# shanpenghui/ExtractORB

Measured on AMD Instinct MI355X. Metric: frames/sec (ORB extract, 640x480x8-level x1000 feat), higher is better.
Workload: dtype u8; 1 GPU; mono640: 640x480 mono stream, 8 levels, 1000 features, synthetic noise frames; variant=noise, nfeatures=1000, nlevels=8, handles_per_gpu=1, parallelism=frames sharded 512/GPU

## Files before the change

### extractorb_amd/csrc/k_pyramid.hip

```cpp
#include <hip/hip_runtime.h>
#include <stdint.h>

#include "orbx_device.hpp"

namespace orbx {

__device__ __forceinline__ int reflect101(int p, int n) {
    p = p < 0 ? -p : p;
    return p >= n ? 2 * (n - 1) - p : p;
}

constexpr int kPyrRows = kResizeTileRows / 4;
constexpr int kTileCols = 64;
constexpr int kTileRowGroups = 4;
constexpr int kTileRows = kPyrRows * kTileRowGroups;

static __host__ __device__ inline int rowDwords(const LevelGeom& g) { return (kPadL - kEdge + g.w + 2 * kEdge + 3) / 4; }

struct SrcView {
    const uint8_t* p;
    long long frame;
    int stride;
    int readableCols;
    int aligned;
};

__device__ __forceinline__ unsigned mulHi24(unsigned a, unsigned b) {
    unsigned r;
    asm("v_mul_hi_u32_u24 %0, %1, %2" : "=v"(r) : "v"(a), "v"(b));
    return r;
}
__device__ __forceinline__ unsigned pkLshr2(unsigned a) {
    unsigned r;
    asm("v_pk_lshrrev_b16 %0, %2, %1" : "=v"(r) : "v"(a), "s"(0x00020002u));
    return r;
}
typedef unsigned short u16x2 __attribute__((ext_vector_type(2)));

template <bool PACKED>
__device__ __forceinline__ void resizeTile(const SrcView& sv, const LevelGeom& d, const ResizeX* __restrict__ xt, const QuadRec* __restrict__ xq,
                                           const ResizeX* __restrict__ yt, const TileFoot ft, uint8_t* __restrict__ pyr,
                                           int tileX, int tileY, int f, uint8_t* tile, int ldsStride) {
    const int tid = threadIdx.x, col = tid & (kTileCols - 1), rgrp = tid / kTileCols;
    const int nd = rowDwords(d), wB = d.w + 2 * kEdge;
// ... 171 lines not shown
extern "C" int orbx_debug_chain_stamps(unsigned long long* out32) { return (int)hipMemcpyFromSymbol(out32, HIP_SYMBOL(g_chainStamps), sizeof(unsigned long long) * 32); }
__device__ unsigned long long g_chainSpans[3 * 2048];
extern "C" int orbx_debug_chain_spans(unsigned long long* out) { return (int)hipMemcpyFromSymbol(out, HIP_SYMBOL(g_chainSpans), sizeof(g_chainSpans)); }
#define CSPAN_BEGIN do { if (tid == 0 && t < 2048) g_chainSpans[3 * t] = __builtin_amdgcn_s_memrealtime(); } while (0)
#define CSPAN_END(lvl) do { if (tid == 0 && t < 2048) { g_chainSpans[3 * t + 1] = __builtin_amdgcn_s_memrealtime(); g_chainSpans[3 * t + 2] = (unsigned long long)(lvl); } } while (0)
#else
#define CSTAMP(i) do {} while (0)
#define CSPAN_BEGIN do {} while (0)
#define CSPAN_END(lvl) do {} while (0)
#endif

template <int T>
__device__ __forceinline__ void chainStep(const uint8_t* S, uint8_t* D, const ChainRegion rs, const ChainRegion rd, const ChainDeal dl, const ResizeX* qrs, const ResizeX* cys,
                                          const int ss, const int ds, const int tid) {
    static_assert(T == 256 || T == 512, "PyrColumn::deal holds the dealing for 256 and 512 deriving threads");
    const int nq = (rd.w + 3) >> 2, nb = dl.nb, blk = (int)(((unsigned)tid * dl.recip) >> 20), x4 = 4 * (tid - blk * nq);
    const int per = dl.per, yb = blk * per, ye = min(yb + per, (int)rd.h);
    if (blk < nb && yb < ye) {
        u16x2 wt[4];
        unsigned sel[4];
        const uint4* qr = (const uint4*)((const QuadRec*)qrs + (x4 >> 2));
        const uint4 q0 = qr[0], q1 = qr[1];
        const unsigned bs = ((const unsigned*)qr)[8];
        sel[0] = q0.x; sel[1] = q0.y; sel[2] = q0.z; sel[3] = q0.w;
        wt[0] = __builtin_bit_cast(u16x2, q1.x); wt[1] = __builtin_bit_cast(u16x2, q1.y); wt[2] = __builtin_bit_cast(u16x2, q1.z); wt[3] = __builtin_bit_cast(u16x2, q1.w);
        const int base = (int)(bs & 0xffffu);
        const unsigned sh = bs >> 16;
        auto hrow = [&](int srow, unsigned (&h)[4]) {
            const unsigned* rp = (const unsigned*)(S + __mul24(srow - rs.y0, ss) + base);
            const unsigned p0 = rp[0], p1 = rp[1], p2 = rp[2];
            const unsigned P0 = __builtin_amdgcn_alignbyte(p1, p0, sh), P1 = __builtin_amdgcn_alignbyte(p2, p1, sh);
#pragma unroll
            for (int k = 0; k < 4; k++)
                h[k] = __builtin_amdgcn_udot2(__builtin_bit_cast(u16x2, __builtin_amdgcn_perm(P1, P0, sel[k])), wt[k], 0u, false) & ~15u;
        };
        unsigned HA[4] = {0, 0, 0, 0}, HB[4] = {0, 0, 0, 0};
// ... 1 lines not shown
        const RowRec* rrs = (const RowRec*)cys;
        for (int y = yb; y < ye; y++) {
            const RowRec rr = rrs[y];
            if (rr.sA != haveA) { hrow(rr.sA, HA); haveA = rr.sA; }
            if (rr.sB != haveB) { hrow(rr.sB, HB); haveB = rr.sB; }
            unsigned t[4];
#pragma unroll
            for (int k = 0; k < 4; k++) t[k] = mulHi24(rr.bA, HA[k]) + mulHi24(rr.bB, HB[k]) + 2u;
            const unsigned u01 = pkLshr2(t[0] | (t[1] << 16)), u23 = pkLshr2(t[2] | (t[3] << 16));
            *(unsigned*)(D + y * ds + x4) = __builtin_amdgcn_perm(u23, u01, 0x06040200u);
        }
    }
}

template <bool PACKED, int T, int TD>
__global__ __launch_bounds__(T) void k_pyr_cols(SrcView img, const PyrColumn* __restrict__ cols, const ColLevels* __restrict__ lvp, int nlevels,
                                                            const ResizeX* __restrict__ colCoef, int coefSlot,
                                                            uint8_t* __restrict__ pyr, int bufEvenBytes, int f0, int nFrames) {
    static_assert(TD <= T && TD % 64 == 0 && (T - TD) % 64 == 0, "roles are whole waves");
    extern __shared__ __align__(16) uint8_t lds[];
    __shared__ __align__(16) ResizeX coef[kChainCoefMax];
    struct LevelOut { ColOwn own; int w, h, stride; long long off; };
    __shared__ LevelOut outOf[kMaxLevels];
    int t, fr;
    if (!xcdChunkFrame(nFrames, t, fr)) return;
    const int f = f0 + fr, tid = threadIdx.x;
    const PyrColumn& pc = cols[t];
    const ColLevels& lv = *lvp;
    const int top = nlevels - 1;
    LevelOut myOut{};
    if (tid < nlevels) myOut = LevelOut{pc.own[tid], lv.w[tid], lv.h[tid], lv.pyrStride[tid], lv.pyrOff[tid] + (long long)f * lv.pyrFrameBytes[tid]};
    CSTAMP(0);
    CSPAN_BEGIN;
    auto bufOf = [&](int j) { return lds + ((j & 1) ? bufEvenBytes : 0); };
    constexpr int kStatic = 8;
    ChainRegion rj[kStatic + 1];
#pragma unroll
    for (int j = 0; j <= kStatic; j++) rj[j] = pc.region[j];
    {
        const ChainRegion r = rj[0];
        const int nDw = r.w >> 2, total = nDw * r.h;
        const uint8_t* src = img.p + (long long)f * img.frame + (long long)r.y0 * img.stride + r.x0;
        unsigned* dst = (unsigned*)bufOf(0);
        constexpr int kLoads = (kChainMaxH0 * kChainMaxW / 4 + T - 1) / T;
        const float inv = __frcp_rn((float)nDw);
        unsigned w[kLoads];
#pragma unroll
        for (int i = 0; i < kLoads; i++) {
            w[i] = 0;
            if (i * T < total) {
            const int idx = min(tid + i * T, total - 1);
            const int row = (int)(((float)idx + 0.5f) * inv), c = idx - row * nDw;
            const uint8_t* q = src + ((unsigned)__mul24(row, img.stride) + 4u * (unsigned)c);
            const int x = r.x0 + 4 * c;
            if (img.aligned && x >= 0 && x + 3 < img.readableCols) w[i] = *(const unsigned*)q;
            else {
#pragma unroll
                for (int b = 0; b < 4; b++) w[i] |= (unsigned)q[reflect101(x + b, img.readableCols) - x] << (8 * b);
            }
            }
        }
        constexpr int kPerThread = (kChainCoefMax + T - 1) / T;
        const int nCoef = pc.nCoef;
        const ResizeX* mine = colCoef + (size_t)t * (size_t)coefSlot;
        ResizeX cv[kPerThread];
#pragma unroll
        for (int k = 0; k < kPerThread; k++) cv[k] = tid + k * T < nCoef ? mine[tid + k * T] : ResizeX{0, 0, 0, 0};
#pragma unroll
        for (int k = 0; k < kPerThread; k++)
            if (tid + k * T < nCoef) coef[tid + k * T] = cv[k];
        if (tid < nlevels) outOf[tid] = myOut;
#pragma unroll
        for (int i = 0; i < kLoads; i++)
            if (tid + i * T < total) dst[tid + i * T] = w[i];
    }
    __syncthreads();
    CSTAMP(1);
    int off = 0;
    auto doLevel = [&](const int j, const ChainRegion rs, const ChainRegion rd) {
        const int ss = (rs.w + 3) & ~3;
        const uint8_t* S = bufOf(j);
        constexpr int TW = TD < T ? T - TD : T;
        if (j < top) {
            const ResizeX* cxs = coef + off;
            const int nqUnits = 6 * ((rd.w + 3) >> 2);
            if (tid < TD) chainStep<TD>(S, bufOf(j + 1), rs, rd, pc.deal[TD == 512][j + 1 < kMaxLevels ? j + 1 : j], cxs, cxs + nqUnits, ss, (rd.w + 3) & ~3, tid);
            off += nqUnits + 2 * rd.h;
        }
        const bool everyone = TD == T || j == top;
        const int wtid = everyone ? tid : tid - TD, wstep = everyone ? T : TW;
        if (wtid >= 0) {
        const LevelOut lo = outOf[j];
        const ColOwn own = lo.own;
        const int w = lo.w, h = lo.h, wB = w + 2 * kEdge;
        uint8_t* out = pyr + lo.off;
        const int stride = lo.stride, nrows = own.r1 - own.r0;
        const int fa = max((int)own.dw0, kPadL / 4), fb = max(fa, min((int)own.dw1, kPadL / 4 + (w >> 2)));
        if (fb > fa && (fb - fa) * nrows <= 2 * wstep) {
            const int ndw = fb - fa, total = ndw * nrows;
            const float inv = __frcp_rn((float)ndw);
            for (int i = wtid; i < total; i += wstep) {
                const int rr = (int)(((float)i + 0.5f) * inv), dw = fa + (i - rr * ndw), row = own.r0 + rr;
                const uint8_t* srow = S + __mul24(reflect101(row - kEdge, h) - rs.y0, ss) - rs.x0;
                *(unsigned*)(out + (long long)row * stride + 4 * dw) = *(const unsigned*)(srow + (4 * dw - kPadL));
            }
        } else if (fb > fa) {
            const int ndw = fb - fa;
            const float rdw = __frcp_rn((float)ndw);
            const int ngrp = max((int)(((float)wstep + 0.5f) * rdw), 1);
            const int per = (int)(((float)(nrows + ngrp - 1) + 0.5f) * __frcp_rn((float)ngrp));
            const int grp = (int)(((float)wtid + 0.5f) * rdw), c = wtid - grp * ndw;
            if (wtid >= 0 && grp < ngrp) {
                const int rA = own.r0 + grp * per, rB = min(rA + per, (int)own.r1);
                const uint8_t* scol = S + (4 * (fa + c) - kPadL - rs.x0);
                uint8_t* ocol = out + 4 * (fa + c);
                auto run = [&](const int r0, const int r1, const int src0, const int sstep) {
                    const uint8_t* sp = scol + __mul24(src0 - rs.y0, ss);
                    uint8_t* op = ocol + (long long)r0 * stride;
                    for (int row = r0; row < r1; row++, op += stride, sp += sstep) *(unsigned*)op = *(const unsigned*)sp;
                };
                const int t1 = min(rB, kEdge), m0 = max(rA, kEdge), m1 = min(rB, kEdge + h), b0 = max(rA, kEdge + h);
                if (rA < t1) run(rA, t1, kEdge - rA, -ss);
                if (m0 < m1) run(m0, m1, m0 - kEdge, ss);
                if (b0 < rB) run(b0, rB, 2 * (h - 1) - (b0 - kEdge), -ss);
            }
        }
        const int nL = fa - own.dw0, nO = nL + (own.dw1 - fb);
        if (nO > 0) {
            const int total = nO * nrows;
            const float inv = __frcp_rn((float)nO);
            for (int i = wtid; i < total; i += wstep) {
                const int rr = (int)(((float)i + 0.5f) * inv), jj = i - rr * nO, dw = jj < nL ? own.dw0 + jj : fb + (jj - nL), row = own.r0 + rr;
                const uint8_t* srow = S + __mul24(reflect101(row - kEdge, h) - rs.y0, ss) - rs.x0;
                const int bc0 = 4 * dw;
                unsigned o = 0;
#pragma unroll
                for (int k = 0; k < 4; k++) {
                    int bx = bc0 + k - (kPadL - kEdge);
                    bx = bx < 0 ? 0 : (bx > wB - 1 ? wB - 1 : bx);
                    o |= (unsigned)srow[reflect101(bx - kEdge, w)] << (8 * k);
                }
                *(unsigned*)(out + (long long)row * stride + bc0) = o;
            }
        }
        }
        __syncthreads();
        CSTAMP(j + 2);
    };
#pragma unroll
    for (int j = 0; j < kStatic; j++)
        if (j <= top) doLevel(j, rj[j], rj[j + 1]);
    for (int j = kStatic; j <= top; j++) doLevel(j, pc.region[j], pc.region[j + 1 < kMaxLevels ? j + 1 : j]);
    CSPAN_END(0);
}

void launchPyrCols(hipStream_t st, const uint8_t* img, long long stride, long long frameStride, int imgW, const PyrColumn* cols, int nCols,
                   const ColLevels* lv, int nlevels, const ResizeX* colCoef, int coefSlot, uint8_t* pyr, int ldsBytes, int bufEvenBytes,
                   bool packed, int shape, int f0, int B) {
    SrcView sv;
    sv.p = img; sv.stride = (int)stride; sv.frame = frameStride; sv.readableCols = imgW;
    sv.aligned = (((uintptr_t)img | (uintptr_t)stride | (uintptr_t)frameStride) & 3) == 0;
#define ORBX_COLS_LAUNCH(P, T, TD) hipLaunchKernelGGL((k_pyr_cols<P, T, TD>), xcdGrid(nCols, B), dim3(T), (size_t)ldsBytes, st, sv, cols, lv, nlevels, colCoef, coefSlot, \
                                                  pyr, bufEvenBytes, f0, B)
    (void)packed;
    if (shape == 6) ORBX_COLS_LAUNCH(true, 1024, 512);
    else if (shape == 4) ORBX_COLS_LAUNCH(true, 768, 256);
    else ORBX_COLS_LAUNCH(true, 512, 256);
#undef ORBX_COLS_LAUNCH
}

void launchPyrFirst(hipStream_t st, const uint8_t* img, long long stride, long long frameStride, const LevelGeom& g0,
                    const LevelGeom* g1, int tilesX0, int tilesY0, int tilesX1, int tilesY1, const ResizeX* xt, const QuadRec* xq,
                    const ResizeX* yt, const TileFoot* foot, uint8_t* pyr, int ldsStride, int ldsRows, bool packed, int f0, int B) {
    SrcView sv;
    sv.p = img; sv.stride = (int)stride; sv.frame = frameStride; sv.readableCols = g0.w;
    sv.aligned = (((uintptr_t)img | (uintptr_t)stride | (uintptr_t)frameStride) & 3) == 0;
    const int n0 = tilesX0 * tilesY0, n1 = g1 ? tilesX1 * tilesY1 : 0;
// ... 15 lines not shown
```

### extractorb_amd/csrc/orbx_api.cpp

```cpp
#include "orbx_internal.hpp"

static_assert(sizeof(orbx_keypoint) == sizeof(Keypoint), "orbx_keypoint layout");
static_assert(sizeof(orbx_proj_query) == sizeof(ProjQuery), "orbx_proj_query layout");

double g_hostT[8];
long g_hostN;
const bool g_hostTiming = getenv("ORBX_HOST_TIMING") && atoi(getenv("ORBX_HOST_TIMING")) != 0;
TestAids g_aids;
const char* const kSlotNames[ORBX_NUM_KERNELS] = {"k_pyr_first", "k_resize", "k_blur", "k_fast",
                                            "k_octree", "k_describe", "memset+copies", "batch_total",
                                            "k_stereo_rows+match+filter", "k_frame_finish+k_search_init+k_search_proj"};
thread_local std::string g_createError;

namespace {
void freeAll(orbx_handle* h) {
    void* dev[] = {h->d_input, h->d_pyr, h->d_blur, h->d_candPos, h->d_candSeg, h->d_cellCount, h->d_cellOff, h->d_nodeOf, h->d_candCount, h->d_sink, h->d_sel, h->d_levelCount,
                   h->d_levelLap, h->d_lap, h->d_lv, h->d_cells, h->d_rx, h->d_ry, h->d_xq, h->d_cols, h->d_colLevels, h->d_colCoef, h->d_foot, h->d_tiles, h->d_laneItem, h->d_out,
                   h->d_octArena, h->d_leafHist, h->d_leafBest, h->d_leafCode, h->d_bowWord, h->d_bowNode, h->d_bowWeight, h->d_rowOff, h->d_sadDist,
                   h->d_nMatched, h->d_rowList, h->d_uRight, h->d_depth, h->d_clock, h->d_sim3Rec, h->d_frustumCounts, h->twoViewWork.prep, h->twoViewWork.first,
                   h->twoViewWork.second, h->twoViewWork.score, h->twoViewWork.mats, h->twoViewWork.inl, h->twoViewWork.counted, h->twoViewWork.cosv, h->sim3SolveWork.prep,
                   h->sim3SolveWork.idx1, h->sim3SolveWork.pts, h->sim3SolveWork.counts, h->sim3SolveWork.its};
    for (void* p : dev) if (p) (void)hipFree(p);
    if (h->evFork) (void)hipEventDestroy(h->evFork);
    if (h->evJoin) (void)hipEventDestroy(h->evJoin);
    if (h->aux) (void)hipStreamDestroy(h->aux);
    if (h->aux2) (void)hipStreamDestroy(h->aux2);
    if (h->probeStream) { (void)hipStreamSynchronize(h->probeStream); (void)hipStreamDestroy(h->probeStream); }
    for (int i = 0; i < 2; i++) { if (h->evPyr[i]) (void)hipEventDestroy(h->evPyr[i]); if (h->evBlur[i]) (void)hipEventDestroy(h->evBlur[i]); if (h->evUp[i]) (void)hipEventDestroy(h->evUp[i]); }
    void* host[] = {h->h_lap, h->h_out, h->h_in, h->h_pyr, h->h_tab};
    for (void* p : host) if (p) (void)hipHostFree(p);
    for (auto& ev : h->pending) { (void)hipEventDestroy(ev.a); (void)hipEventDestroy(ev.b); }
    if (h->ownStream && h->stream) (void)hipStreamDestroy(h->stream);
// ... 55 lines not shown
    stage(h->d_lv, g.lv, sizeof(LevelGeom) * g.nlevels);
    stage(h->d_cells, g.cells.data(), sizeof(CellDesc) * g.cells.size());
    size_t fo = 0;
    for (int l = 1; l < g.nlevels; l++) {
        footOff[l] = fo;
        if (fo + g.foot[l].size() > h->footCap) return fail(h, ORBX_ERR_IMAGE_TOO_LARGE, "tile footprint table does not fit");
        stage(h->d_foot + fo, g.foot[l].data(), sizeof(TileFoot) * g.foot[l].size());
        fo += g.foot[l].size();
    }
    {
        size_t n = 0, nc = 0;
        for (FrameGeom::ColumnSet& cs : g.colSets) {
            if (n + cs.columns.size() > h->colsCap || nc + cs.coef.size() > h->colCoefCap) cs.fit = false;
            if (!cs.fit) continue;
            stage(h->d_cols + n, cs.columns.data(), sizeof(PyrColumn) * cs.columns.size());
            stage(h->d_colCoef + nc, cs.coef.data(), sizeof(ResizeX) * cs.coef.size());
            const size_t slot = &cs - g.colSets.data();
            colsOff[slot] = n;
            colCoefOff[slot] = nc;
            n += cs.columns.size();
            nc += cs.coef.size();
        }
        ColLevels c{};
        c.nlevels = g.nlevels;
        for (int l = 0; l < g.nlevels; l++) {
            c.w[l] = g.lv[l].w; c.h[l] = g.lv[l].h; c.pyrStride[l] = g.lv[l].pyrStride; c.rxOff[l] = g.lv[l].rxOff; c.ryOff[l] = g.lv[l].ryOff;
            c.pyrOff[l] = g.lv[l].pyrOff; c.pyrFrameBytes[l] = g.lv[l].pyrFrameBytes;
        }
        stage(h->d_colLevels, &c, sizeof(c));
    }
// ... 76 lines not shown
    auto pollute = [&](hipStream_t st) { if (h->ldsPollute >= 0) launchLdsPollute(st, lp.numCUs, h->ldsPollute, h->d_sink); };
    auto blurTable = [&](hipStream_t st, int v, int blockRows, int f0, int Bn) {
        launchBlur(st, h->d_tiles + gp.blurItemOff[v], h->d_laneItem + gp.blurLaneOff[v], gp.nBlurLanes[v], blockRows, h->d_lv, h->d_pyr, h->d_blur, f0, Bn);
    };
    bool blurJoin[2] = {false, false};
    int blurF0[2] = {0, 0}, blurBn[2] = {0, 0};
    auto front = [&](hipStream_t st, int f0, int Bn) {
        const FrontPlan fp = planFront(g, gp, lp, state, bp, Bn);
        h->lastPyrCut = fp.cut >= 0 ? g.colSets[fp.cut].px : 0;
        h->lastPyrForm = fp.pyrForm();
        if (fp.cut >= 0) {
            const FrameGeom::ColumnSet& cs = g.colSets[fp.cut];
            Prof p(h, S_RESIZE, st);
            h->lastKernel[S_RESIZE] = fp.resizeKernel;
            pollute(st);
            launchPyrCols(st, d_imgs, stride, frameStride, g.lv[0].w, h->d_cols + h->colsOff[fp.cut], (int)cs.columns.size(), h->d_colLevels, g.nlevels,
                          h->d_colCoef + h->colCoefOff[fp.cut], cs.coefSlot, h->d_pyr, cs.ldsBytes, cs.evenBytes,
                          g.colsPacked && !lp.resizeBytewise, fp.colsShape, f0, Bn);
        } else {
            {
                Prof p(h, S_LEVEL0, st);
                pollute(st);
                launchPyrFirst(st, d_imgs, stride, frameStride, g.lv[0], g.nlevels > 1 ? &g.lv[1] : nullptr, g.tilesX[0], g.tilesY[0],
                               g.tilesX[1], g.tilesY[1], h->d_rx + h->rxOff[1], h->d_xq + h->xqOff[1], h->d_ry + h->ryOff[1], h->d_foot + h->footOff[1], h->d_pyr,
                               g.tileLdsStride, g.tileLdsRows, g.packedTaps[1] && !lp.resizeBytewise, f0, Bn);
            }
            for (int l = 2; l < g.nlevels; l++) {
                Prof p(h, S_RESIZE, st);
                h->lastKernel[S_RESIZE] = fp.resizeKernel;
                pollute(st);
                launchResize(st, g.lv[l - 1], g.lv[l], g.tilesX[l], g.tilesY[l], h->d_rx + h->rxOff[l], h->d_xq + h->xqOff[l], h->d_ry + h->ryOff[l],
// ... 332 lines not shown
    h->colPx = envInt("ORBX_PYR_COL_PX", 0);
    h->launch.fastWide = envInt("ORBX_FAST_WIDE", -1);
    h->launch.patchBlur = envInt("ORBX_PATCH_BLUR", -1);
    h->launch.blurSplit = envInt("ORBX_BLUR_SPLIT", -1);
    h->sharedUploadBytes = g_aids.sharedUploadBytes;
    h->twoEyesWalk = g_aids.twoEyesWalk == 1;
    h->describeSums = g_aids.describeSums == 0 || g_aids.describeSums == 1 ? g_aids.describeSums : -1;
    h->twoEyesBowStage = g_aids.twoEyesBowStage != 0;
    h->launch.colsShape = g_aids.colsShape == 1 || g_aids.colsShape == 4 || g_aids.colsShape == 6 ? g_aids.colsShape : -1;
    h->colsCap = 0;
    for (int px : kColPx) h->colsCap += (size_t)((max_width + px / 2) / px + 1) * ((max_height + px / 2) / px + 1);
    h->colCoefCap = (h->colsCap + h->colsCap / 8 + 16) * (size_t)kChainCoefMax * 5 / 8;
    h->colsCap = roomy(h->colsCap);
    CREATE_ALLOC(h->d_colCoef, sizeof(ResizeX) * h->colCoefCap);
    CREATE_ALLOC(h->d_cols, sizeof(PyrColumn) * h->colsCap);
    CREATE_ALLOC(h->d_colLevels, sizeof(ColLevels));
    h->footCap = roomy((size_t)((max_width + 38 + 255) / 256 + 1) * ((max_height + 38 + 31) / 32 + 1) * nlevels);
    CREATE_ALLOC(h->d_foot, sizeof(TileFoot) * h->footCap);
    h->outBytes = outLayout(max_batch, h->outCap, nlevels).all;
    CREATE_ALLOC(h->d_out, h->outBytes);
    h->testFailAfterFast = g_aids.failAfterFast != 0;
    g_aids.failAfterFast = 0;
    h->zeroCopy = envInt("ORBX_ZERO_COPY", 1) != 0;
    CREATE_TRY(hipHostMalloc(&h->h_lap, sizeof(int) * 2 * max_batch));
    CREATE_TRY(hipStreamCreateWithFlags(&h->aux, hipStreamNonBlocking));
    CREATE_TRY(hipStreamCreateWithFlags(&h->aux2, hipStreamNonBlocking));
    for (int i = 0; i < 2; i++) { CREATE_TRY(hipEventCreateWithFlags(&h->evPyr[i], hipEventDisableTiming)); CREATE_TRY(hipEventCreateWithFlags(&h->evBlur[i], hipEventDisableTiming)); }
    for (int i = 0; i < 2; i++) CREATE_TRY(hipEventCreateWithFlags(&h->evUp[i], hipEventDisableTiming));
    CREATE_TRY(hipEventCreateWithFlags(&h->evFork, hipEventDisableTiming));
    CREATE_TRY(hipEventCreateWithFlags(&h->evJoin, hipEventDisableTiming));
// ... 309 lines not shown
```

### extractorb_amd/csrc/orbx_device.hpp

```cpp
#pragma once
#include <stddef.h>
#include <stdint.h>

namespace orbx {

constexpr int kEdge = 19;
constexpr int kPadL = 32;
constexpr int kHalfPatch = 15;
constexpr int kPatch = 31;
constexpr int kMaxLevels = 16;
constexpr int kCellW = 30;
constexpr int kMinBorder = kEdge - 3;
constexpr int kGridCols = 64, kGridRows = 48, kGridCells = kGridCols * kGridRows;


struct Keypoint {
    float x, y, size, angle, response;
    int octave, class_id;
};
static_assert(sizeof(Keypoint) == 28, "cv::KeyPoint layout");

template <bool BIG> struct CandFmt;
template <> struct CandFmt<false> {
    typedef unsigned T;
// ... 116 lines not shown
struct RowRec { unsigned bA, bB; int sA, sB; };
ORBX_HD inline RowRec makeRowRec(const ResizeX& cy) {
    const bool swap = ((cy.sx0 ^ cy.sx1) & 1) && (cy.sx0 & 1);
    const unsigned b0 = (unsigned)(unsigned short)cy.a0 << 12, b1 = (unsigned)(unsigned short)cy.a1 << 12;
    return swap ? RowRec{b1, b0, cy.sx1, cy.sx0} : RowRec{b0, b1, cy.sx0, cy.sx1};
}
struct ColOwn { short dw0, dw1, r0, r1; };
struct ChainDeal { unsigned recip; short nb, per; };
inline ChainDeal makeChainDeal(int w, int h, int TD) {
    const int nq = (w + 3) >> 2;
    if (nq <= 0 || h <= 0) return ChainDeal{0u, 0, 0};
    const int nb = TD / nq;
    return ChainDeal{(unsigned)(((1u << 20) + nq - 1) / nq), (short)nb, (short)(nb > 0 ? (h + nb - 1) / nb : 0)};
}
struct PyrColumn { ChainRegion region[kMaxLevels]; ColOwn own[kMaxLevels]; ChainDeal deal[2][kMaxLevels]; int nCoef, pad; };
struct ColLevels {
    int nlevels, pad;
    int w[kMaxLevels], h[kMaxLevels], pyrStride[kMaxLevels], rxOff[kMaxLevels], ryOff[kMaxLevels];
    long long pyrOff[kMaxLevels], pyrFrameBytes[kMaxLevels];
};

struct DescLevel {
    int selOff, w, h, pyrStride, blurStride, patchSize;
    float scale;
    int pad;
    long long pyrOff, pyrFrameBytes, blurOff, blurFrameBytes;
};
static_assert(sizeof(DescLevel) == 64, "one line per level");
struct DescLevels {
    int firstSlot[kMaxLevels];
// ... 55 lines not shown
```

### extractorb_amd/csrc/orbx_geometry.hpp

```cpp
#pragma once
#include <cmath>
#include <cstdint>
#include <algorithm>
#include <cstring>
#include <string>
#include <vector>

#include "orbx_device.hpp"

namespace orbx {

inline int roundHalfEven(float v) { return (int)std::lrintf(v); }
inline int roundHalfEven(double v) { return (int)std::lrint(v); }
inline int roundUp(int v, int m) { return (v + m - 1) / m * m; }

struct ScaleTables {
    int nlevels = 0;
    float scale[kMaxLevels] = {}, invScale[kMaxLevels] = {}, sigma2[kMaxLevels] = {}, invSigma2[kMaxLevels] = {};
    int quota[kMaxLevels] = {};
    int patchSize[kMaxLevels] = {};
    int umax[kHalfPatch + 1] = {};
};

inline ScaleTables makeScaleTables(int nfeatures, float scaleFactorF, int nlevels) {
// ... 67 lines not shown
    std::vector<ResizeX> ry[kMaxLevels];
    std::vector<TileFoot> foot[kMaxLevels];
    int tilesX[kMaxLevels] = {}, tilesY[kMaxLevels] = {};
    int tileLdsStride = 16, tileLdsRows = 1;
    bool packedTaps[kMaxLevels] = {};
    std::vector<QuadRec> xq[kMaxLevels];
    long long pyrBytesPerFrame = 0, blurBytesPerFrame = 0;
    long long candPerFrame = 0;
    int selPerFrame = 0;
    int maxRoiW = 0, maxRoiH = 0;
    int maxNodes = 0;
    long long sumPixels = 0;
    struct ColumnSet {
        int px = 0, RX = 0, RY = 0;
        std::vector<PyrColumn> columns;
        bool fit = false;
        int ldsBytes = 0, evenBytes = 0;
        int coefSlot = 0;
        std::vector<ResizeX> coef;
    };
    std::vector<ColumnSet> colSets;
    bool colsPacked = false;
    bool big = false;
};
constexpr int kColPx[] = {40, 56, 80, 112};
#ifndef ORBX_COL_EDGE_NUM
#define ORBX_COL_EDGE_NUM 3
#define ORBX_COL_EDGE_DEN 5
#endif
constexpr int kColEdgeNum = ORBX_COL_EDGE_NUM, kColEdgeDen = ORBX_COL_EDGE_DEN;

inline std::string makeFrameGeom(const ScaleTables& t, int rows, int cols, FrameGeom& g, int colPx = 0) {
    g = FrameGeom();
    g.rows = rows; g.cols = cols; g.nlevels = t.nlevels;
    for (int l = 0; l < t.nlevels; l++) {
        LevelGeom& L = g.lv[l];
        L.w = roundHalfEven((float)cols * t.invScale[l]);
        L.h = roundHalfEven((float)rows * t.invScale[l]);
        const int maxBorderX = L.w - kEdge + 3, maxBorderY = L.h - kEdge + 3;
// ... 188 lines not shown
                    int w = nx1 - nx0 + 1;
                    if (l == 0) w = (w + 3) & ~3;
                    const int hh = ny1 - ny0 + 1, bytes = ((w + 3) & ~3) * hh;
                    c.region[l] = ChainRegion{(short)nx0, (short)ny0, (short)w, (short)hh};
                    c.deal[0][l] = makeChainDeal(w, hh, 256); c.deal[1][l] = makeChainDeal(w, hh, 512);
                    if (w > kChainMaxW || (l == 0 && bytes > kChainMaxW * kChainMaxH0)) fits = false;
                    if (l & 1) maxOdd = std::max(maxOdd, bytes); else maxEven = std::max(maxEven, bytes);
                    if (l >= 1) coefs += 6 * ((w + 3) >> 2) + 2 * hh;
                    x0 = nx0; x1 = std::min(nx0 + w - 1, L.w - 1); y0 = ny0; y1 = ny1;
                    if (l == 0) x1 = nx1;
                }
                if (coefs > kChainCoefMax) fits = false;
                c.nCoef = coefs;
                if (coefs > cs.coefSlot) cs.coefSlot = coefs;
                cs.columns.push_back(c);
            }
        cs.coefSlot = (cs.coefSlot + 7) & ~7;
        if (fits) {
            cs.coef.assign(cs.columns.size() * (size_t)cs.coefSlot, ResizeX{0, 0, 0, 0});
            for (size_t i = 0; i < cs.columns.size(); i++) {
                ResizeX* q = cs.coef.data() + i * (size_t)cs.coefSlot;
                for (int l = 1; l <= top; l++) {
                    const ChainRegion& r = cs.columns[i].region[l];
                    const ChainRegion& rs = cs.columns[i].region[l - 1];
                    for (int x4 = 0; x4 < r.w; x4 += 4) {
                        QuadRec qr{};
                        int c0[4], c1[4], lo = 1 << 30;
                        for (int k = 0; k < 4; k++) {
                            const ResizeX& cx = g.rx[l][refl(r.x0 + std::min(x4 + k, r.w - 1), g.lv[l].w)];
                            c0[k] = cx.sx0 - rs.x0; c1[k] = cx.sx1 - rs.x0;
// ... 94 lines not shown
```

### extractorb_amd/csrc/orbx_internal.hpp

```cpp
#pragma once
#include <hip/hip_runtime.h>

#include <algorithm>
#include <cmath>
#include <cstdio>
#include <cstdlib>
#include <cstring>
#include <ctime>
#include <mutex>
#include <string>
#include <vector>

#include "orbx.h"
#include "orbx_entry.hpp"
#include "orbx_geometry.hpp"
#include "orbx_batch_plan.hpp"
#include "orbx_params.hpp"

namespace orbx {
void launchPyrFirst(hipStream_t, const uint8_t*, long long, long long, const LevelGeom&, const LevelGeom*, int, int, int, int,
                    const ResizeX*, const QuadRec*, const ResizeX*, const TileFoot*, uint8_t*, int, int, bool, int, int);
void launchResize(hipStream_t, const LevelGeom&, const LevelGeom&, int, int, const ResizeX*, const QuadRec*, const ResizeX*, const TileFoot*,
                  uint8_t*, int, int, bool, int, int);
size_t bowMatchLdsBytes(int capacity, bool stageDesc);
// ... 8 lines not shown
void launchSearchTriangulationTwoEyes(hipStream_t, const uint32_t*, const uint32_t*, const int*, const uint8_t*, const uint8_t*, const float*, const Keypoint*, const uint8_t*, const int*, const TriMatchTwoEyesParams&, bool, int*, int*, int*, int);
void launchKb8Unproject(hipStream_t, const float*, const float*, int, float*);
void launchKb8Triangulate(hipStream_t, const float*, const float*, const Kb8TriangulateParams&, float*, float*);
int stereoFisheyeTiles(int capacity);
void launchStereoFisheye(hipStream_t, const Keypoint*, const uint8_t*, const int*, const int*, const StereoFisheyeParams&, int*, int*, float*, float*, int*, int*, int);
int newMapPointsTiles(int listCapacity);
void launchNewMapPoints(hipStream_t, bool, const int*, const int*, const float*, const Keypoint*, const Keypoint*, const float*, const float*, const int*, const NewMapPointsParams&, uint8_t*, float*, int*, uint8_t*, uint8_t*, int);
void launchMapPointUpdate(hipStream_t, bool, const MapPointUpdateArrays&, const MapPointUpdateParams&);
void launchTwoView(hipStream_t, const Keypoint*, const int*, int*, int*, const int*, const TwoViewParams&, const TvWork&, void*, float*, uint8_t*, int);
void launchSim3Solve(hipStream_t, const void*, const float*, const float*, const int*, const int*, const int*, const Sim3SolveParams&, const SsWork&, void*, uint8_t*, int, int);
void launchPoseOptimization(hipStream_t, const void*, const Keypoint*, const int*, const float*, const int*, const float*, const PoseOptParams&, float*, uint8_t*, void*, int);
size_t sim3SettleLdsBytes(int capacity, int mpCapacity);
size_t sim3RecordBytes();
void launchSim3Search(hipStream_t, const float*, const float*, const float*, const uint8_t*, const int*, const uint8_t*, const float*, const Keypoint*, const uint8_t*, const int*, const int*, const int*, const uint8_t*, const Sim3SearchParams&, void*, int*, int*, int*, uint8_t*, int*, int);
void launchLdsPollute(hipStream_t, int, int, unsigned*);
void launchPyrCols(hipStream_t, const uint8_t*, long long, long long, int, const PyrColumn*, int, const ColLevels*, int, const ResizeX*, int, uint8_t*, int, int, bool, int, int, int);
void launchBlur(hipStream_t, const BlurItem*, const unsigned short*, int, int, const LevelGeom*, const uint8_t*, uint8_t*, int, int);
void launchFast(hipStream_t, const CellDesc*, int, const LevelGeom*, int, const uint8_t*, int, int, unsigned*, unsigned*,
                int, int, int, int, const BlurItem*, const unsigned short*, int, uint8_t*, LeafTables, bool, bool);
bool fastCanCarryBlur(int, int);
size_t octreeLdsBytes(int M, int P, int R, int XT);
void launchOctree(hipStream_t, const LevelGeom*, int, const CellDesc*, int, const unsigned*, const unsigned*, int*, unsigned*,
                  unsigned*, unsigned short*, uint2*, int, int*, int*, const int*, int, int, int, int, const int*, bool, int, int, uint8_t*, LeafTables, bool);
void launchDescribe(hipStream_t, const DescLevels&, const uint8_t*, const uint8_t*, const uint2*, int, const int*,
                    const int*, Keypoint*, uint8_t*, int, int*, int*, Keypoint*, int*, bool, int, int, int, int, int, int, int);
bool checkUmax(const int* umax16);
void describeTables(unsigned* pb384, unsigned* plain256);
hipError_t runPackedSelfTest(hipStream_t, unsigned*, unsigned*);
void launchFrameFinish(hipStream_t, const Keypoint*, const int*, const FrameFinishParams&, Keypoint*, int*, int*, int*, int);
void launchStereo(hipStream_t, const LevelGeom*, const uint8_t*, const Keypoint*, const uint8_t*, const int*, const StereoParams&,
                  int, int*, unsigned short*, float*, float*, int*, int*, int);
// ... 70 lines not shown
    unsigned *d_candPos = nullptr, *d_candSeg = nullptr;
    unsigned* d_cellCount = nullptr;
    int* d_cellOff = nullptr;
    unsigned short* d_nodeOf = nullptr;
    unsigned* d_candCount = nullptr;
    unsigned* d_sink = nullptr;
    uint2* d_sel = nullptr;
    int *d_levelCount = nullptr, *d_levelLap = nullptr, *d_lap = nullptr;
    LevelGeom* d_lv = nullptr;
    DescLevels descLevels = {};
    CellDesc* d_cells = nullptr;
    ResizeX *d_rx = nullptr, *d_ry = nullptr;
    QuadRec* d_xq = nullptr;
    size_t xqCap = 0, xqOff[kMaxLevels] = {};
    PyrColumn* d_cols = nullptr;
    size_t colsCap = 0, colsOff[4] = {};
    ResizeX* d_colCoef = nullptr;
    size_t colCoefCap = 0, colCoefOff[4] = {};
    ColLevels* d_colLevels = nullptr;
    int colPx = 0;
    TileFoot* d_foot = nullptr;
    size_t footCap = 0, footOff[kMaxLevels] = {};
    BlurItem* d_tiles = nullptr;
    unsigned short* d_laneItem = nullptr;
    size_t laneCap = 0;
    size_t rxOff[kMaxLevels] = {}, ryOff[kMaxLevels] = {};
    size_t octArenaSlice = 0;
    uint8_t* d_octArena = nullptr;
    int octM = 0, octP = 0, octR = 0, octXT = 0;
    int* d_leafHist = nullptr;
// ... 171 lines not shown
```

Baseline: 323,200 frames/s.

## Precompute per-column load and write dealing tables on host for pyramid kernel

```diff
diff --git a/extractorb_amd/csrc/k_pyramid.hip b/extractorb_amd/csrc/k_pyramid.hip
--- a/extractorb_amd/csrc/k_pyramid.hip
+++ b/extractorb_amd/csrc/k_pyramid.hip
@@ -28,6 +28,11 @@
 __device__ __forceinline__ unsigned mulHi24(unsigned a, unsigned b) {
     unsigned r;
     asm("v_mul_hi_u32_u24 %0, %1, %2" : "=v"(r) : "v"(a), "v"(b));
+    return r;
+}
+__device__ __forceinline__ unsigned mulU24(unsigned a, unsigned b) {
+    unsigned r;
+    asm("v_mul_u32_u24 %0, %1, %2" : "=v"(r) : "v"(a), "v"(b));
     return r;
 }
 __device__ __forceinline__ unsigned pkLshr2(unsigned a) {
@@ -229,12 +234,12 @@
 __device__ __forceinline__ void chainStep(const uint8_t* S, uint8_t* D, const ChainRegion rs, const ChainRegion rd, const ChainDeal dl, const ResizeX* qrs, const ResizeX* cys,
                                           const int ss, const int ds, const int tid) {
     static_assert(T == 256 || T == 512, "PyrColumn::deal holds the dealing for 256 and 512 deriving threads");
-    const int nq = (rd.w + 3) >> 2, nb = dl.nb, blk = (int)(((unsigned)tid * dl.recip) >> 20), x4 = 4 * (tid - blk * nq);
-    const int per = dl.per, yb = blk * per, ye = min(yb + per, (int)rd.h);
+    const int nq = (rd.w + 3) >> 2, nb = dl.nb, blk = (int)(mulU24((unsigned)tid, dl.recip) >> 20), x4 = 4 * (tid - __mul24(blk, nq));
+    const int per = dl.per, yb = __mul24(blk, per), ye = min(yb + per, (int)rd.h);
     if (blk < nb && yb < ye) {
         u16x2 wt[4];
         unsigned sel[4];
-        const uint4* qr = (const uint4*)((const QuadRec*)qrs + (x4 >> 2));
+        const uint4* qr = (const uint4*)((const uint8_t*)qrs + __mul24(x4 >> 2, (int)sizeof(QuadRec)));
         const uint4 q0 = qr[0], q1 = qr[1];
         const unsigned bs = ((const unsigned*)qr)[8];
         sel[0] = q0.x; sel[1] = q0.y; sel[2] = q0.z; sel[3] = q0.w;
@@ -266,22 +271,31 @@
 }
 
 template <bool PACKED, int T, int TD>
-__global__ __launch_bounds__(T) void k_pyr_cols(SrcView img, const PyrColumn* __restrict__ cols, const ColLevels* __restrict__ lvp, int nlevels,
+__global__ __launch_bounds__(T) void k_pyr_cols(SrcView img, const PyrColumn* __restrict__ cols, const ColDeal* __restrict__ deals, const ColLevels* __restrict__ lvp, int nlevels,
                                                             const ResizeX* __restrict__ colCoef, int coefSlot,
                                                             uint8_t* __restrict__ pyr, int bufEvenBytes, int f0, int nFrames) {
     static_assert(TD <= T && TD % 64 == 0 && (T - TD) % 64 == 0, "roles are whole waves");
     extern __shared__ __align__(16) uint8_t lds[];
     __shared__ __align__(16) ResizeX coef[kChainCoefMax];
-    struct LevelOut { ColOwn own; int w, h, stride; long long off; };
-    __shared__ LevelOut outOf[kMaxLevels];
+    struct LevelOut { ColWrite wr; int dw0, r0, r1, w; int h, stride; long long off; };
+    static_assert(sizeof(LevelOut) == 80, "five 16-byte LDS reads");
+    __shared__ __align__(16) LevelOut outOf[kMaxLevels];
     int t, fr;
     if (!xcdChunkFrame(nFrames, t, fr)) return;
     const int f = f0 + fr, tid = threadIdx.x;
     const PyrColumn& pc = cols[t];
+    const ColDeal& dl = deals[t];
     const ColLevels& lv = *lvp;
     const int top = nlevels - 1;
+    constexpr int TW = TD < T ? T - TD : T;
     LevelOut myOut{};
-    if (tid < nlevels) myOut = LevelOut{pc.own[tid], lv.w[tid], lv.h[tid], lv.pyrStride[tid], lv.pyrOff[tid] + (long long)f * lv.pyrFrameBytes[tid]};
+    if (tid < nlevels) {
+        const ColOwn own = pc.own[tid];
+        const uint4* wp = (const uint4*)&dl.write[tid == top ? colWriterSlot(T) : colWriterSlot(TW)][tid];
+        const uint4 w0 = wp[0], w1 = wp[1], w2 = wp[2];
+        myOut = LevelOut{ColWrite{(int)w0.x, (int)w0.y, (int)w0.z, (int)w0.w, w1.x, (int)w1.y, (int)w1.z, (int)w1.w, (int)w2.x, (int)w2.y, w2.z, (int)w2.w},
+                         own.dw0, own.r0, own.r1, lv.w[tid], lv.h[tid], lv.pyrStride[tid], lv.pyrOff[tid] + (long long)f * lv.pyrFrameBytes[tid]};
+    }
     CSTAMP(0);
     CSPAN_BEGIN;
     auto bufOf = [&](int j) { return lds + ((j & 1) ? bufEvenBytes : 0); };
@@ -289,27 +303,40 @@
     ChainRegion rj[kStatic + 1];
 #pragma unroll
     for (int j = 0; j <= kStatic; j++) rj[j] = pc.region[j];
+    ChainDeal dj[kStatic + 1];
+#pragma unroll
+    for (int j = 1; j <= kStatic; j++) dj[j] = pc.deal[TD == 512][j];
     {
         const ChainRegion r = rj[0];
-        const int nDw = r.w >> 2, total = nDw * r.h;
+        const ColLoad ld = dl.load[colThreadSlot(T)];
+        const int nDw = r.w >> 2, rpp = ld.rowsPerPass, passes = ld.passes;
         const uint8_t* src = img.p + (long long)f * img.frame + (long long)r.y0 * img.stride + r.x0;
         unsigned* dst = (unsigned*)bufOf(0);
-        constexpr int kLoads = (kChainMaxH0 * kChainMaxW / 4 + T - 1) / T;
-        const float inv = __frcp_rn((float)nDw);
+        constexpr int kLoads = chainLoadPasses(T);
+        const int row0 = (int)(mulU24((unsigned)tid, ld.recip) >> 20), c = tid - __mul24(row0, nDw);
+        const int left = row0 < rpp ? r.h - row0 : 0;
+        const int x = r.x0 + 4 * c;
+        const uint8_t* q0 = src + ((unsigned)__mul24(row0, img.stride) + 4u * (unsigned)c);
+        const unsigned gstep = (unsigned)(rpp * img.stride);
+        const int lstep = rpp * nDw;
         unsigned w[kLoads];
-#pragma unroll
-        for (int i = 0; i < kLoads; i++) {
-            w[i] = 0;
-            if (i * T < total) {
-            const int idx = min(tid + i * T, total - 1);
-            const int row = (int)(((float)idx + 0.5f) * inv), c = idx - row * nDw;
-            const uint8_t* q = src + ((unsigned)__mul24(row, img.stride) + 4u * (unsigned)c);
-            const int x = r.x0 + 4 * c;
-            if (img.aligned && x >= 0 && x + 3 < img.readableCols) w[i] = *(const unsigned*)q;
-            else {
-#pragma unroll
-                for (int b = 0; b < 4; b++) w[i] |= (unsigned)q[reflect101(x + b, img.readableCols) - x] << (8 * b);
-            }
+        if (img.aligned && x + 3 < img.readableCols) {
+#pragma unroll
+            for (int i = 0; i < kLoads; i++, q0 += gstep) {
+                w[i] = 0;
+                if (i < passes && i * rpp < left) w[i] = *(const unsigned*)q0;
+            }
+        } else {
+            int bo[4];
+#pragma unroll
+            for (int b = 0; b < 4; b++) bo[b] = reflect101(x + b, img.readableCols) - x;
+#pragma unroll
+            for (int i = 0; i < kLoads; i++, q0 += gstep) {
+                w[i] = 0;
+                if (i < passes && i * rpp < left) {
+#pragma unroll
+                    for (int b = 0; b < 4; b++) w[i] |= (unsigned)q0[bo[b]] << (8 * b);
+                }
             }
         }
         constexpr int kPerThread = (kChainCoefMax + T - 1) / T;
@@ -323,53 +350,46 @@
             if (tid + k * T < nCoef) coef[tid + k * T] = cv[k];
         if (tid < nlevels) outOf[tid] = myOut;
 #pragma unroll
-        for (int i = 0; i < kLoads; i++)
-            if (tid + i * T < total) dst[tid + i * T] = w[i];
+        for (int i = 0, li = tid; i < kLoads; i++, li += lstep)
+            if (i < passes && i * rpp < left) dst[li] = w[i];
     }
     __syncthreads();
     CSTAMP(1);
     int off = 0;
-    auto doLevel = [&](const int j, const ChainRegion rs, const ChainRegion rd) {
+    auto doLevel = [&](const int j, const ChainRegion rs, const ChainRegion rd, const ChainDeal dn) {
         const int ss = (rs.w + 3) & ~3;
         const uint8_t* S = bufOf(j);
-        constexpr int TW = TD < T ? T - TD : T;
         if (j < top) {
             const ResizeX* cxs = coef + off;
             const int nqUnits = 6 * ((rd.w + 3) >> 2);
-            if (tid < TD) chainStep<TD>(S, bufOf(j + 1), rs, rd, pc.deal[TD == 512][j + 1 < kMaxLevels ? j + 1 : j], cxs, cxs + nqUnits, ss, (rd.w + 3) & ~3, tid);
+            if (tid < TD) chainStep<TD>(S, bufOf(j + 1), rs, rd, dn, cxs, cxs + nqUnits, ss, (rd.w + 3) & ~3, tid);
             off += nqUnits + 2 * rd.h;
         }
         const bool everyone = TD == T || j == top;
         const int wtid = everyone ? tid : tid - TD, wstep = everyone ? T : TW;
         if (wtid >= 0) {
         const LevelOut lo = outOf[j];
-        const ColOwn own = lo.own;
+        const ColWrite wr = lo.wr;
         const int w = lo.w, h = lo.h, wB = w + 2 * kEdge;
-        uint8_t* out = pyr + lo.off;
-        const int stride = lo.stride, nrows = own.r1 - own.r0;
-        const int fa = max((int)own.dw0, kPadL / 4), fb = max(fa, min((int)own.dw1, kPadL / 4 + (w >> 2)));
-        if (fb > fa && (fb - fa) * nrows <= 2 * wstep) {
-            const int ndw = fb - fa, total = ndw * nrows;
-            const float inv = __frcp_rn((float)ndw);
-            for (int i = wtid; i < total; i += wstep) {
-                const int rr = (int)(((float)i + 0.5f) * inv), dw = fa + (i - rr * ndw), row = own.r0 + rr;
+        uint8_t* out = pyr + (((unsigned long long)(unsigned)__builtin_amdgcn_readfirstlane((int)(lo.off >> 32)) << 32) | (unsigned)__builtin_amdgcn_readfirstlane((int)lo.off));
+        const int stride = __builtin_amdgcn_readfirstlane(lo.stride), r0 = lo.r0, r1 = lo.r1;
+        const int form = __builtin_amdgcn_readfirstlane(wr.form);
+        if (form == 1) {
+            for (int i = wtid; i < wr.total; i += wstep) {
+                const int rr = (int)(mulU24((unsigned)i, wr.rdw) >> 20), dw = wr.fa + (i - __mul24(rr, wr.ndw)), row = r0 + rr;
                 const uint8_t* srow = S + __mul24(reflect101(row - kEdge, h) - rs.y0, ss) - rs.x0;
-                *(unsigned*)(out + (long long)row * stride + 4 * dw) = *(const unsigned*)(srow + (4 * dw - kPadL));
-            }
-        } else if (fb > fa) {
-            const int ndw = fb - fa;
-            const float rdw = __frcp_rn((float)ndw);
-            const int ngrp = max((int)(((float)wstep + 0.5f) * rdw), 1);
-            const int per = (int)(((float)(nrows + ngrp - 1) + 0.5f) * __frcp_rn((float)ngrp));
-            const int grp = (int)(((float)wtid + 0.5f) * rdw), c = wtid - grp * ndw;
-            if (wtid >= 0 && grp < ngrp) {
-                const int rA = own.r0 + grp * per, rB = min(rA + per, (int)own.r1);
-                const uint8_t* scol = S + (4 * (fa + c) - kPadL - rs.x0);
-                uint8_t* ocol = out + 4 * (fa + c);
-                auto run = [&](const int r0, const int r1, const int src0, const int sstep) {
+                *(unsigned*)(out + (unsigned)(__mul24(row, stride) + 4 * dw)) = *(const unsigned*)(srow + (4 * dw - kPadL));
+            }
+        } else if (form == 2) {
+            const int grp = (int)(mulU24((unsigned)wtid, wr.rdw) >> 20), c = wtid - __mul24(grp, wr.ndw);
+            if (grp < wr.ngrp) {
+                const int rA = r0 + __mul24(grp, wr.per), rB = min(rA + wr.per, r1);
+                const uint8_t* scol = S + (4 * (wr.fa + c) - kPadL - rs.x0);
+                auto run = [&](const int ra, const int rb, const int src0, const int sstep) {
                     const uint8_t* sp = scol + __mul24(src0 - rs.y0, ss);
-                    uint8_t* op = ocol + (long long)r0 * stride;
-                    for (int row = r0; row < r1; row++, op += stride, sp += sstep) *(unsigned*)op = *(const unsigned*)sp;
+                    unsigned o = (unsigned)(__mul24(ra, stride) + 4 * (wr.fa + c));
+                    const unsigned oEnd = o + (unsigned)__mul24(rb - ra, stride);
+                    for (; o != oEnd; o += (unsigned)stride, sp += sstep) *(unsigned*)(out + o) = *(const unsigned*)sp;
                 };
                 const int t1 = min(rB, kEdge), m0 = max(rA, kEdge), m1 = min(rB, kEdge + h), b0 = max(rA, kEdge + h);
                 if (rA < t1) run(rA, t1, kEdge - rA, -ss);
@@ -377,12 +397,9 @@
                 if (b0 < rB) run(b0, rB, 2 * (h - 1) - (b0 - kEdge), -ss);
             }
         }
-        const int nL = fa - own.dw0, nO = nL + (own.dw1 - fb);
-        if (nO > 0) {
-            const int total = nO * nrows;
-            const float inv = __frcp_rn((float)nO);
-            for (int i = wtid; i < total; i += wstep) {
-                const int rr = (int)(((float)i + 0.5f) * inv), jj = i - rr * nO, dw = jj < nL ? own.dw0 + jj : fb + (jj - nL), row = own.r0 + rr;
+        if (__builtin_amdgcn_readfirstlane(wr.nO) > 0) {
+            for (int i = wtid; i < wr.totalO; i += wstep) {
+                const int rr = (int)(mulU24((unsigned)i, wr.rO) >> 20), jj = i - __mul24(rr, wr.nO), dw = jj < wr.nL ? lo.dw0 + jj : wr.fb + (jj - wr.nL), row = r0 + rr;
                 const uint8_t* srow = S + __mul24(reflect101(row - kEdge, h) - rs.y0, ss) - rs.x0;
                 const int bc0 = 4 * dw;
                 unsigned o = 0;
@@ -392,7 +409,7 @@
                     bx = bx < 0 ? 0 : (bx > wB - 1 ? wB - 1 : bx);
                     o |= (unsigned)srow[reflect101(bx - kEdge, w)] << (8 * k);
                 }
-                *(unsigned*)(out + (long long)row * stride + bc0) = o;
+                *(unsigned*)(out + (unsigned)(__mul24(row, stride) + bc0)) = o;
             }
         }
         }
@@ -401,18 +418,18 @@
     };
 #pragma unroll
     for (int j = 0; j < kStatic; j++)
-        if (j <= top) doLevel(j, rj[j], rj[j + 1]);
-    for (int j = kStatic; j <= top; j++) doLevel(j, pc.region[j], pc.region[j + 1 < kMaxLevels ? j + 1 : j]);
+        if (j <= top) doLevel(j, rj[j], rj[j + 1], dj[j + 1]);
+    for (int j = kStatic; j <= top; j++) doLevel(j, pc.region[j], pc.region[j + 1 < kMaxLevels ? j + 1 : j], pc.deal[TD == 512][j + 1 < kMaxLevels ? j + 1 : j]);
     CSPAN_END(0);
 }
 
-void launchPyrCols(hipStream_t st, const uint8_t* img, long long stride, long long frameStride, int imgW, const PyrColumn* cols, int nCols,
+void launchPyrCols(hipStream_t st, const uint8_t* img, long long stride, long long frameStride, int imgW, const PyrColumn* cols, const ColDeal* deals, int nCols,
                    const ColLevels* lv, int nlevels, const ResizeX* colCoef, int coefSlot, uint8_t* pyr, int ldsBytes, int bufEvenBytes,
                    bool packed, int shape, int f0, int B) {
     SrcView sv;
     sv.p = img; sv.stride = (int)stride; sv.frame = frameStride; sv.readableCols = imgW;
     sv.aligned = (((uintptr_t)img | (uintptr_t)stride | (uintptr_t)frameStride) & 3) == 0;
-#define ORBX_COLS_LAUNCH(P, T, TD) hipLaunchKernelGGL((k_pyr_cols<P, T, TD>), xcdGrid(nCols, B), dim3(T), (size_t)ldsBytes, st, sv, cols, lv, nlevels, colCoef, coefSlot, \
+#define ORBX_COLS_LAUNCH(P, T, TD) hipLaunchKernelGGL((k_pyr_cols<P, T, TD>), xcdGrid(nCols, B), dim3(T), (size_t)ldsBytes, st, sv, cols, deals, lv, nlevels, colCoef, coefSlot, \
                                                   pyr, bufEvenBytes, f0, B)
     (void)packed;
     if (shape == 6) ORBX_COLS_LAUNCH(true, 1024, 512);
diff --git a/extractorb_amd/csrc/orbx_api.cpp b/extractorb_amd/csrc/orbx_api.cpp
--- a/extractorb_amd/csrc/orbx_api.cpp
+++ b/extractorb_amd/csrc/orbx_api.cpp
@@ -15,7 +15,7 @@
 namespace {
 void freeAll(orbx_handle* h) {
     void* dev[] = {h->d_input, h->d_pyr, h->d_blur, h->d_candPos, h->d_candSeg, h->d_cellCount, h->d_cellOff, h->d_nodeOf, h->d_candCount, h->d_sink, h->d_sel, h->d_levelCount,
-                   h->d_levelLap, h->d_lap, h->d_lv, h->d_cells, h->d_rx, h->d_ry, h->d_xq, h->d_cols, h->d_colLevels, h->d_colCoef, h->d_foot, h->d_tiles, h->d_laneItem, h->d_out,
+                   h->d_levelLap, h->d_lap, h->d_lv, h->d_cells, h->d_rx, h->d_ry, h->d_xq, h->d_cols, h->d_colDeal, h->d_colLevels, h->d_colCoef, h->d_foot, h->d_tiles, h->d_laneItem, h->d_out,
                    h->d_octArena, h->d_leafHist, h->d_leafBest, h->d_leafCode, h->d_bowWord, h->d_bowNode, h->d_bowWeight, h->d_rowOff, h->d_sadDist,
                    h->d_nMatched, h->d_rowList, h->d_uRight, h->d_depth, h->d_clock, h->d_sim3Rec, h->d_frustumCounts, h->twoViewWork.prep, h->twoViewWork.first,
                    h->twoViewWork.second, h->twoViewWork.score, h->twoViewWork.mats, h->twoViewWork.inl, h->twoViewWork.counted, h->twoViewWork.cosv, h->sim3SolveWork.prep,
@@ -101,6 +101,7 @@
             if (n + cs.columns.size() > h->colsCap || nc + cs.coef.size() > h->colCoefCap) cs.fit = false;
             if (!cs.fit) continue;
             stage(h->d_cols + n, cs.columns.data(), sizeof(PyrColumn) * cs.columns.size());
+            stage(h->d_colDeal + n, cs.deals.data(), sizeof(ColDeal) * cs.deals.size());
             stage(h->d_colCoef + nc, cs.coef.data(), sizeof(ResizeX) * cs.coef.size());
             const size_t slot = &cs - g.colSets.data();
             colsOff[slot] = n;
@@ -207,7 +208,7 @@
             Prof p(h, S_RESIZE, st);
             h->lastKernel[S_RESIZE] = fp.resizeKernel;
             pollute(st);
-            launchPyrCols(st, d_imgs, stride, frameStride, g.lv[0].w, h->d_cols + h->colsOff[fp.cut], (int)cs.columns.size(), h->d_colLevels, g.nlevels,
+            launchPyrCols(st, d_imgs, stride, frameStride, g.lv[0].w, h->d_cols + h->colsOff[fp.cut], h->d_colDeal + h->colsOff[fp.cut], (int)cs.columns.size(), h->d_colLevels, g.nlevels,
                           h->d_colCoef + h->colCoefOff[fp.cut], cs.coefSlot, h->d_pyr, cs.ldsBytes, cs.evenBytes,
                           g.colsPacked && !lp.resizeBytewise, fp.colsShape, f0, Bn);
         } else {
@@ -570,6 +571,7 @@
     h->colsCap = roomy(h->colsCap);
     CREATE_ALLOC(h->d_colCoef, sizeof(ResizeX) * h->colCoefCap);
     CREATE_ALLOC(h->d_cols, sizeof(PyrColumn) * h->colsCap);
+    CREATE_ALLOC(h->d_colDeal, sizeof(ColDeal) * h->colsCap);
     CREATE_ALLOC(h->d_colLevels, sizeof(ColLevels));
     h->footCap = roomy((size_t)((max_width + 38 + 255) / 256 + 1) * ((max_height + 38 + 31) / 32 + 1) * nlevels);
     CREATE_ALLOC(h->d_foot, sizeof(TileFoot) * h->footCap);
diff --git a/extractorb_amd/csrc/orbx_device.hpp b/extractorb_amd/csrc/orbx_device.hpp
--- a/extractorb_amd/csrc/orbx_device.hpp
+++ b/extractorb_amd/csrc/orbx_device.hpp
@@ -154,6 +154,16 @@
     return ChainDeal{(unsigned)(((1u << 20) + nq - 1) / nq), (short)nb, (short)(nb > 0 ? (h + nb - 1) / nb : 0)};
 }
 struct PyrColumn { ChainRegion region[kMaxLevels]; ColOwn own[kMaxLevels]; ChainDeal deal[2][kMaxLevels]; int nCoef, pad; };
+constexpr int kColThreads[3] = {512, 768, 1024};
+constexpr int kColWriters[4] = {256, 512, 768, 1024};
+constexpr int colThreadSlot(int T) { return T / 256 - 2; }
+constexpr int colWriterSlot(int n) { return n / 256 - 1; }
+constexpr int chainLoadPasses(int T) { return (kChainMaxH0 * kChainMaxW / 4 + T - 1) / T + 2; }
+struct ColLoad { unsigned recip; short rowsPerPass, passes; };
+struct ColWrite { int form, fa, fb, ndw; unsigned rdw; int ngrp, per, total; int nL, nO; unsigned rO; int totalO; };
+static_assert(sizeof(ColWrite) == 48, "three 16-byte loads");
+struct ColDeal { ColLoad load[3]; int pad[2]; ColWrite write[4][kMaxLevels]; };
+static_assert(sizeof(ColDeal) % 16 == 0 && offsetof(ColDeal, write) % 16 == 0, "ColWrite records are read as 16-byte vectors");
 struct ColLevels {
     int nlevels, pad;
     int w[kMaxLevels], h[kMaxLevels], pyrStride[kMaxLevels], rxOff[kMaxLevels], ryOff[kMaxLevels];
diff --git a/extractorb_amd/csrc/orbx_geometry.hpp b/extractorb_amd/csrc/orbx_geometry.hpp
--- a/extractorb_amd/csrc/orbx_geometry.hpp
+++ b/extractorb_amd/csrc/orbx_geometry.hpp
@@ -105,6 +105,7 @@
     struct ColumnSet {
         int px = 0, RX = 0, RY = 0;
         std::vector<PyrColumn> columns;
+        std::vector<ColDeal> deals;
         bool fit = false;
         int ldsBytes = 0, evenBytes = 0;
         int coefSlot = 0;
@@ -114,6 +115,51 @@
     bool colsPacked = false;
     bool big = false;
 };
+inline unsigned scaledRecip(int n) { return n > 0 ? (unsigned)(((1u << 20) + n - 1) / n) : 0u; }
+inline bool scaledRecipExact(int n, long long count) {
+    if (count <= 0) return true;
+    if (n <= 0 || count > (1 << 24)) return false;
+    const long long recip = scaledRecip(n), e = (long long)n * recip - (1LL << 20);
+    return (count - 1) * e < (1LL << 20) && (count - 1) * recip < (1LL << 32);
+}
+inline ColLoad makeColLoad(int w, int h, int T, bool& ok) {
+    const int nDw = w >> 2;
+    if (nDw < 1 || h < 1 || nDw > T || !scaledRecipExact(nDw, T)) { ok = false; return ColLoad{0u, 0, 0}; }
+    const int rpp = T / nDw, passes = (h + rpp - 1) / rpp;
+    if (passes > chainLoadPasses(T)) ok = false;
+    return ColLoad{scaledRecip(nDw), (short)rpp, (short)passes};
+}
+inline ColWrite makeColWrite(const ColOwn own, int w, int h, int writers, bool& ok) {
+    ColWrite r{};
+    (void)h;
+    const int nrows = own.r1 - own.r0;
+    if (nrows <= 0 || own.dw1 <= own.dw0) return r;
+    r.fa = std::max((int)own.dw0, kPadL / 4);
+    r.fb = std::max(r.fa, std::min((int)own.dw1, kPadL / 4 + (w >> 2)));
+    r.ndw = r.fb - r.fa;
+    if (r.ndw > 0) {
+        r.rdw = scaledRecip(r.ndw);
+        if (r.ndw * nrows <= 2 * writers) {
+            r.form = 1;
+            r.total = r.ndw * nrows;
+            if (!scaledRecipExact(r.ndw, r.total)) ok = false;
+        } else {
+            r.form = 2;
+            r.ngrp = std::max(writers / r.ndw, 1);
+            r.per = (nrows + r.ngrp - 1) / r.ngrp;
+            if (r.ndw > writers || !scaledRecipExact(r.ndw, writers)) ok = false;
+        }
+    }
+    r.nL = r.fa - own.dw0;
+    r.nO = r.nL + (own.dw1 - r.fb);
+    if (r.nO > 0) {
+        r.rO = scaledRecip(r.nO);
+        r.totalO = r.nO * nrows;
+        if (!scaledRecipExact(r.nO, r.totalO)) ok = false;
+    }
+    return r;
+}
+
 constexpr int kColPx[] = {40, 56, 80, 112};
 #ifndef ORBX_COL_EDGE_NUM
 #define ORBX_COL_EDGE_NUM 3
@@ -332,6 +378,11 @@
                 c.nCoef = coefs;
                 if (coefs > cs.coefSlot) cs.coefSlot = coefs;
                 cs.columns.push_back(c);
+                ColDeal d{};
+                for (int v = 0; v < 3; v++) d.load[v] = makeColLoad(c.region[0].w, c.region[0].h, kColThreads[v], fits);
+                for (int v = 0; v < 4; v++)
+                    for (int l = 0; l <= top; l++) d.write[v][l] = makeColWrite(c.own[l], g.lv[l].w, g.lv[l].h, kColWriters[v], fits);
+                cs.deals.push_back(d);
             }
         cs.coefSlot = (cs.coefSlot + 7) & ~7;
         if (fits) {
diff --git a/extractorb_amd/csrc/orbx_internal.hpp b/extractorb_amd/csrc/orbx_internal.hpp
--- a/extractorb_amd/csrc/orbx_internal.hpp
+++ b/extractorb_amd/csrc/orbx_internal.hpp
@@ -46,7 +46,7 @@
 size_t sim3RecordBytes();
 void launchSim3Search(hipStream_t, const float*, const float*, const float*, const uint8_t*, const int*, const uint8_t*, const float*, const Keypoint*, const uint8_t*, const int*, const int*, const int*, const uint8_t*, const Sim3SearchParams&, void*, int*, int*, int*, uint8_t*, int*, int);
 void launchLdsPollute(hipStream_t, int, int, unsigned*);
-void launchPyrCols(hipStream_t, const uint8_t*, long long, long long, int, const PyrColumn*, int, const ColLevels*, int, const ResizeX*, int, uint8_t*, int, int, bool, int, int, int);
+void launchPyrCols(hipStream_t, const uint8_t*, long long, long long, int, const PyrColumn*, const ColDeal*, int, const ColLevels*, int, const ResizeX*, int, uint8_t*, int, int, bool, int, int, int);
 void launchBlur(hipStream_t, const BlurItem*, const unsigned short*, int, int, const LevelGeom*, const uint8_t*, uint8_t*, int, int);
 void launchFast(hipStream_t, const CellDesc*, int, const LevelGeom*, int, const uint8_t*, int, int, unsigned*, unsigned*,
                 int, int, int, int, const BlurItem*, const unsigned short*, int, uint8_t*, LeafTables, bool, bool);
@@ -147,6 +147,7 @@
     QuadRec* d_xq = nullptr;
     size_t xqCap = 0, xqOff[kMaxLevels] = {};
     PyrColumn* d_cols = nullptr;
+    ColDeal* d_colDeal = nullptr;
     size_t colsCap = 0, colsOff[4] = {};
     ResizeX* d_colCoef = nullptr;
     size_t colCoefCap = 0, colCoefOff[4] = {};
```

New measurement: 326,100 frames/s (median of 6 runs). No clear change (+0.9%).
